# XiaoshuiHuang/GMF

Hardware: AMD Instinct MI355X
Metric: correspondences/sec (whole node) (higher is better)
Workload: dtype f32 (split-fp16 MFMA operands, fp32 accumulate; the cross products of the attention's two contractions, S = K Q'^T and O = P V, on block-scaled e4m3 operands wherever the device-side score guard allows)

## Files before the change

### gmf_amd/csrc/enc_common.hpp

```cpp
#pragma once
#include "mfma_core.hpp"
#include "launchers.hpp"
#include "kv_share_layout.hpp"

namespace gmf {

constexpr int C = 128;
constexpr int CF = C / 2;
constexpr int DH = 64;
constexpr int DHF = DH / 2;
constexpr int FFH = 512;
constexpr int kWavesPerWG = 4;

GMF_DEVINL void load_vec_block(float (&v)[16], const float* __restrict__ vec, int mb, int h) {
  const float4* p = reinterpret_cast<const float4*>(vec + 32 * mb) + h;
#pragma unroll
  for (int q = 0; q < 4; ++q) {
    const float4 t = p[2 * q];
    v[4 * q + 0] = t.x; v[4 * q + 1] = t.y; v[4 * q + 2] = t.z; v[4 * q + 3] = t.w;
  }
}

GMF_DEVINL void store_block_p32(float* __restrict__ tile_base, int mb, const float (&t)[16], int lane) {
  float4* p = reinterpret_cast<float4*>(tile_base) + (4 * mb) * 64 + lane;
// ... 209 lines not shown
  for (int s = 0; s < NS; ++s) mma3(acc, lw[(0 * NS + s) * 64], lw[(1 * NS + s) * 64], x.h[s], x.l[s]);
}

template <int NS>
GMF_DEVINL void mma_xw_h2(f32x16& acc, const f16x8* lw, const FragH2<NS>& x) {
#pragma unroll
  for (int s = 0; s < NS; ++s) mma3(acc, x.h[s], x.l[s], lw[(0 * NS + s) * 64], lw[(1 * NS + s) * 64]);
}

template <int NP>
GMF_DEVINL void mma_np(f32x16& acc, f16x8 ah, f16x8 al, f16x8 bh, f16x8 bl) {
  if (NP == 3) mma3(acc, ah, al, bh, bl);
  else acc = mfma_h16(ah, bh, acc);
}
template <int NS, int NP>
GMF_DEVINL void mma_wx_h2n(f32x16& acc, const f16x8* lw, const FragH2<NS>& x) {
#pragma unroll
  for (int s = 0; s < NS; ++s) {
    if (NP == 3) mma3(acc, lw[(0 * NS + s) * 64], lw[(1 * NS + s) * 64], x.h[s], x.l[s]);
    else acc = mfma_h16(lw[(0 * NS + s) * 64], x.h[s], acc);
  }
}
template <int NS, int NP>
GMF_DEVINL void mma_xw_h2n(f32x16& acc, const f16x8* lw, const FragH2<NS>& x) {
#pragma unroll
  for (int s = 0; s < NS; ++s) {
    if (NP == 3) mma3(acc, x.h[s], x.l[s], lw[(0 * NS + s) * 64], lw[(1 * NS + s) * 64]);
    else acc = mfma_h16(x.h[s], lw[(0 * NS + s) * 64], acc);
  }
}

GMF_DEVINL const f16x8* as_h2(const float4* p) { return reinterpret_cast<const f16x8*>(p); }

GMF_DEVINL float gelu_erf(float x) { return 0.5f * x * (1.0f + erff(x * 0.70710678118654752440f)); }

GMF_DEVINL float erf_bf(float a) {
  const float t = fabsf(a), s = a * a;
  float r = fmaf(-1.72853470e-5f, t, 3.83197126e-4f);
  const float u = fmaf(-3.88396438e-3f, t, 2.42546219e-2f);
  r = fmaf(r, s, u);
  r = fmaf(r, t, -1.06777877e-1f);
  r = fmaf(r, t, -6.34846687e-1f);
  r = fmaf(r, t, -1.28717512e-1f);
  r = fmaf(r, t, -t);
  const float big = 1.0f - __builtin_amdgcn_exp2f(r * 1.4426950408889634f);
  float q = -5.96761703e-4f;
  q = fmaf(q, s, 4.99119423e-3f);
  q = fmaf(q, s, -2.67681349e-2f);
  q = fmaf(q, s, 1.12819925e-1f);
  q = fmaf(q, s, -3.76125336e-1f);
  q = fmaf(q, s, 1.28379166e-1f);
  const float small = fmaf(q, t, t);
  return copysignf(t > 0.927734375f ? big : small, a);
}
GMF_DEVINL float gelu_erf_bf(float x) { return 0.5f * x * (1.0f + erf_bf(x * 0.70710678118654752440f)); }

GMF_DEVINL float gelu_erf_1r(float x) {
  const float ax = fabsf(x);
  const float t = fminf(ax * 0.70710678118654752440f, 4.3f);
  float p = 1.160468673e-05f;
  p = fmaf(p, t, -1.529631263e-04f);
  p = fmaf(p, t, 8.482293342e-04f);
  p = fmaf(p, t, -2.274774713e-03f);
  p = fmaf(p, t, 8.479235839e-05f);
  p = fmaf(p, t, 2.772448584e-02f);
  p = fmaf(p, t, -1.483079195e-01f);
  p = fmaf(p, t, -9.184429049e-01f);
  p = fmaf(p, t, -1.627907276e+00f);
  const float e = __builtin_amdgcn_exp2f(p * t);
  return fmaf(-0.5f * ax, e, fmaxf(x, 0.f));
}


GMF_DEVINL float len_diff(float a2, float b2) { return sqrt_cr(a2) - sqrt_cr(b2); }

GMF_DEVINL float compat_times(const float4* lp, int jl, const float (&si)[3], const float (&ti)[3], float inv_sig2, float sc) {
  const float4 a = lp[2 * jl], b = lp[2 * jl + 1];
  const float ax = si[0] - a.x, ay = si[1] - a.y, az = si[2] - a.z;
  const float bx = ti[0] - b.x, by = ti[1] - b.y, bz = ti[2] - b.z;
  const float d = len_diff(fmaf(az, az, fmaf(ay, ay, ax * ax)), fmaf(bz, bz, fmaf(by, by, bx * bx)));
  return fmaxf(1.0f - d * d * inv_sig2, 0.f) * sc;
}

constexpr int kJPerWave = 8;

constexpr int kCompatLdsFloats = 4 * 32 * 33;
template <int FMT>
GMF_DEVINL void compat_build_body(float* tr, const int I, const int by, const int pair, const float* __restrict__ pts8,
                                  float* __restrict__ c_dense, int N, int tiles, float inv_sig2, const PairTab* __restrict__ ptab) {
  const int lane = threadIdx.x & 63, h = lane >> 5, i = lane & 31;
  const int wave = __builtin_amdgcn_readfirstlane(threadIdx.x >> 6);
  const int tiles_p = (pair_rows(ptab, pair, N) + 31) >> 5;
  if (I >= tiles_p) return;
  const size_t pbase = (size_t)pair * tiles;
  float si[3], ti[3];
  {
    const float4* pp = reinterpret_cast<const float4*>(pts8 + (pbase * 32 + (size_t)I * 32 + i) * 8);
    const float4 a = pp[0], b = pp[1];
    si[0] = a.x; si[1] = a.y; si[2] = a.z; ti[0] = b.x; ti[1] = b.y; ti[2] = b.z;
  }
  constexpr int kTile16 = FMT ? 128 : 256;
  float4* const cbase = reinterpret_cast<float4*>(c_dense) + pbase * (size_t)tiles * kTile16 + lane;
  float4* const crow = cbase + (size_t)I * tiles * kTile16;
  auto store_tile = [&](float4* ct, const float (&c)[16]) {
    if (FMT == 1) {
#pragma unroll
      for (int q2 = 0; q2 < 2; ++q2) {
        f16x8 hv;
#pragma unroll
        for (int e = 0; e < 8; ++e) hv[e] = (_Float16)c[8 * q2 + e];
        ct[q2 * 64] = __builtin_bit_cast(float4, hv);
      }
    } else if (FMT == 2) {
#pragma unroll
      for (int q2 = 0; q2 < 2; ++q2) {
        unsigned wv[4];
        auto enc = [](float cv) { return (unsigned)__builtin_rintf(cv * 65535.0f); };
#pragma unroll
        for (int e = 0; e < 8; e += 2) wv[e >> 1] = enc(c[8 * q2 + e]) | (enc(c[8 * q2 + e + 1]) << 16);
        ct[q2 * 64] = make_float4(__uint_as_float(wv[0]), __uint_as_float(wv[1]), __uint_as_float(wv[2]), __uint_as_float(wv[3]));
      }
    } else {
#pragma unroll
      for (int q = 0; q < 4; ++q) ct[q * 64] = make_float4(c[4 * q], c[4 * q + 1], c[4 * q + 2], c[4 * q + 3]);
    }
  };
  float* const mt = tr + wave * 32 * 33;
  const int j0 = (by * 4 + wave) * kJPerWave;
  for (int J = max(j0, I); J < min(tiles_p, j0 + kJPerWave); ++J) {
    const float4* lp = reinterpret_cast<const float4*>(pts8 + (pbase * 32 + (size_t)J * 32) * 8) + 8 * h;
    float c[16];
#pragma unroll
    for (int r = 0; r < 16; ++r) c[r] = compat_times(lp, 8 * (r >> 2) + (r & 3), si, ti, inv_sig2, 1.0f);
    store_tile(crow + (size_t)J * kTile16, c);
    if (J > I) {
#pragma unroll
      for (int r = 0; r < 16; ++r) mt[i * 33 + 8 * (r >> 2) + 4 * h + (r & 3)] = c[r];
      asm volatile("s_waitcnt lgkmcnt(0)" ::: "memory");
      float d[16];
#pragma unroll
      for (int r = 0; r < 16; ++r) d[r] = mt[(8 * (r >> 2) + 4 * h + (r & 3)) * 33 + i];
      store_tile(cbase + ((size_t)J * tiles + I) * kTile16, d);
      asm volatile("s_waitcnt lgkmcnt(0)" ::: "memory");
    }
  }
}

GMF_DEVINL void pack_pts8_body(const long idx, const float* __restrict__ src, const float* __restrict__ tgt, float* __restrict__ dst,
                               int N, int Npad, long total, const PairTab* __restrict__ ptab, unsigned* __restrict__ zero_words,
                               int n_zero) {
  if (zero_words && idx < n_zero) zero_words[idx] = 0u;
  if (idx >= total) return;
  const int row = idx % Npad;
  const long b = idx / Npad;
  float4 a = make_float4(0.f, 0.f, 0.f, 0.f), c = a;
  if (row < pair_rows(ptab, (int)b, N)) {
    const size_t r0 = pair_row0(ptab, (int)b, N) + row;
    const float* ps = src + r0 * 3;
    const float* pt = tgt + r0 * 3;
    a = make_float4(ps[0], ps[1], ps[2], 0.f);
    c = make_float4(pt[0], pt[1], pt[2], 0.f);
  }
  reinterpret_cast<float4*>(dst)[2 * idx] = a;
  reinterpret_cast<float4*>(dst)[2 * idx + 1] = c;
}


}
```

### gmf_amd/csrc/encoder_kernels.hip

```cpp
#include <algorithm>
#include <type_traits>
#include "enc_common.hpp"
#include "enc_ff.hpp"

namespace gmf {

template <int MODE>
__global__ void __launch_bounds__(256, 2)
k_front(const float* __restrict__ in, const float* __restrict__ wst, const float* __restrict__ vecs,
        float* __restrict__ f_out, float* __restrict__ q_out, float* __restrict__ k_out,
        float* __restrict__ v_out, int N, int tiles) {
  __shared__ __attribute__((aligned(16))) float lds[2 * kStageFloats];
  const int lane = threadIdx.x & 63, wave = threadIdx.x >> 6, h = lane >> 5, i = lane & 31;
  const int pair = blockIdx.y;
  const int tile_raw = blockIdx.x * kWavesPerWG + wave;
  const bool active = tile_raw < tiles;
  const int tile = active ? tile_raw : tiles - 1;
  const size_t toff = ((size_t)pair * tiles + tile) * (32 * C);

  constexpr bool FIRST = (MODE == 1);
  StageStream ss;
  if (MODE == 2) ss.init(lds, lds + kStageFloats, wave, kWavesPerWG, lane, wst + 4 * kStageFloats, 12);
  else ss.init(lds, lds + kStageFloats, wave, kWavesPerWG, lane, wst, 16);
  ss.prime();
// ... 343 lines not shown
    for (int r = 0; r < 16; ++r) { x[r] = __builtin_amdgcn_exp2f(x[r] - m_off); ls += x[r]; }
    l_half = fmaf(l_half, alpha, ls);
    if (__any(moved)) {
#pragma unroll
      for (int db = 0; db < 4; ++db)
#pragma unroll
        for (int r = 0; r < 16; ++r) oacc[db][r] *= alpha;
    }
#pragma unroll
    for (int s2 = 0; s2 < 2; ++s2) {
      f16x8 ph, pl;
      split8h(&x[8 * s2], ph, pl);
#pragma unroll
      for (int db = 0; db < 4; ++db) {
        const int slot = 2 * db + s2;
        const f16x8 vh = lv[(0 * 8 + slot) * 64], vl = lv[(1 * 8 + slot) * 64];
        mma3(oacc[db], vh, vl, ph, pl);
      }
    }
  };
  for (int t = 0; t < tiles; t += 2) {
    tile_step(t, c_a, c_b);
    if (t + 1 < tiles) tile_step(t + 1, c_b, c_a);
  }

  float o[CF];
  {
    const float inv = 1.0f / xhalf_sum(l_half);
#pragma unroll
    for (int db = 0; db < 4; ++db)
#pragma unroll
      for (int r = 0; r < 16; ++r) o[16 * db + r] = oacc[db][r] * inv;
  }
  __syncthreads();
  StageStream ss;
  ss.init(lds, lds + kStageFloats, wave, WAVES, lane, wst, 5);
  ss.prime();
  float m1[DHF], m2[DHF];
#pragma unroll
  for (int mb = 0; mb < 2; ++mb) {
    const float4* lw = ss.acquire();
    f32x16 acc = zero16();
    mma_wx<CF>(acc, lw, o);
    float b[16];
    load_vec_block(b, vecs, mb, h);
#pragma unroll
    for (int r = 0; r < 16; ++r) m1[16 * mb + r] = relu_nan(acc[r] + b[r]);
  }
  {
    const float4* lw = ss.acquire();
#pragma unroll
    for (int mb = 0; mb < 2; ++mb) {
      f32x16 acc = zero16();
      mma_wx<DHF>(acc, lw + mb * (32 * DH / 4), m1);
      float b[16];
      load_vec_block(b, vecs + 64, mb, h);
#pragma unroll
      for (int r = 0; r < 16; ++r) m2[16 * mb + r] = relu_nan(acc[r] + b[r]);
    }
  }
#pragma unroll
  for (int st = 0; st < 2; ++st) {
    const float4* lw = ss.acquire();
#pragma unroll
    for (int hb = 0; hb < 2; ++hb) {
      const int mb = 2 * st + hb;
      f32x16 acc = zero16();
      mma_wx<DHF>(acc, lw + hb * (32 * DH / 4), m2);
      float b[16], fz[16], t[16];
      load_vec_block(b, vecs + 128, mb, h);
      load_block_p32(fz, fus + toff, mb, lane);
#pragma unroll
      for (int r = 0; r < 16; ++r) t[r] = acc[r] + b[r] + fz[r];
      if (active) store_block_p32(out + toff, mb, t, lane);
    }
  }
}

template <int FMT>
__global__ void __launch_bounds__(256)
k_compat_build(const float* __restrict__ pts8, float* __restrict__ c_dense, int N, int tiles, float inv_sig2,
               const PairTab* __restrict__ ptab) {
  __shared__ float tr[kCompatLdsFloats];
  compat_build_body<FMT>(tr, blockIdx.x, blockIdx.y, blockIdx.z, pts8, c_dense, N, tiles, inv_sig2, ptab);
}

GMF_DEVINL f32x16 mma3_part(int u, f32x16 acc, f16x8 ah, f16x8 al, f16x8 bh, f16x8 bl) {
  switch (u) {
    case 0: return mfma_h16(al, bh, acc);
    case 1: return mfma_h16(ah, bl, acc);
    default: return mfma_h16(ah, bh, acc);
  }
}


struct FusTile {
  const float* tile;
  GMF_DEVINL void load(float (&fz)[16], int mb, int lane, int h) const { load_block_p32(fz, tile, mb, lane); }
};

struct FusRegs {
  const float (&f)[CF];
  GMF_DEVINL void load(float (&fz)[16], int mb, int lane, int h) const {
#pragma unroll
    for (int r = 0; r < 16; ++r) fz[r] = f[16 * mb + r];
  }
};

constexpr int kTailVecFloats = 3 * C;
GMF_DEVINL void stage_tail_vecs(float* lvec, const float* __restrict__ vecs, const float* __restrict__ next_bias, int wave, int lane) {
  if (wave == 0) dma_piece_1k(vecs, lvec, lane);
  if (wave == 1 && next_bias && lane < 32) dma_piece_1k(next_bias, lvec + 2 * C, lane);
}

template <bool NEXT_PCN, class Stages, class Fus>
GMF_DEVINL void scattn_epilogue_h2(const float (&o)[CF], const bool active, Stages& ss, const float* __restrict__ vecs,
                                   const Fus& fus_tile, float* __restrict__ out_tile, const int lane, const int h,
                                   const float* __restrict__ next_bias = nullptr,
                                   unsigned* __restrict__ stat_next = nullptr, const int pair = 0, const bool row_valid = false) {
    FragH2<8> ox, featx;
    FragH2<4> m1x, m2x;
    if (active) ox.set(o);
#pragma unroll
    for (int mb = 0; mb < 2; ++mb) {
      const f16x8* lw = as_h2(ss.acquire());
      if (!active) continue;
      f32x16 acc = zero16();
      mma_wx_h2<8>(acc, lw, ox);
      float b[16], t1[16];
      load_vec_block(b, vecs, mb, h);
#pragma unroll
      for (int r = 0; r < 16; ++r) t1[r] = relu_nan(fmaf(acc[r], kH2Inv, b[r]));
      m1x.set_block(mb, t1);
    }
    {
      const f16x8* lw = as_h2(ss.acquire());
#pragma unroll
      for (int mb = 0; mb < 2; ++mb) {
        if (!active) continue;
        f32x16 acc = zero16();
        mma_wx_h2<4>(acc, lw + mb * (2 * 4 * 64), m1x);
        float b[16], t2[16];
        load_vec_block(b, vecs + 64, mb, h);
#pragma unroll
        for (int r = 0; r < 16; ++r) t2[r] = relu_nan(fmaf(acc[r], kH2Inv, b[r]));
        m2x.set_block(mb, t2);
      }
    }
#pragma unroll
    for (int st = 0; st < 2; ++st) {
      const f16x8* lw = as_h2(ss.acquire());
#pragma unroll
      for (int hb = 0; hb < 2; ++hb) {
        if (!active) continue;
        const int mb = 2 * st + hb;
        f32x16 acc = zero16();
        mma_wx_h2<4>(acc, lw + hb * (2 * 4 * 64), m2x);
        float b[16], fz[16], tt[16];
        load_vec_block(b, vecs + 128, mb, h);
        fus_tile.load(fz, mb, lane, h);
#pragma unroll
        for (int r = 0; r < 16; ++r) tt[r] = fmaf(acc[r], kH2Inv, b[r]) + fz[r];
        if (NEXT_PCN) featx.set_block(mb, tt);
        else if (active) store_block_p32(out_tile, mb, tt, lane);
      }
    }
    if (NEXT_PCN) {
// ... 1446 lines not shown
  const long b = bt / tiles;
  const int row = tile * 32 + (lane & 31);
  const int k0 = 8 * g + 4 * (lane >> 5);
  float4 v = make_float4(0.f, 0.f, 0.f, 0.f);
  if (row < pair_rows(ptab, (int)b, n_rows)) {
    const float* p = src + (ptab ? (long)ptab[b].row0 * sr : b * sb) + (long)row * sr + (long)k0 * sk;
    v = make_float4(p[0], p[sk], p[2 * sk], p[3 * sk]);
  }
  reinterpret_cast<float4*>(dst)[idx] = v;
}

__global__ void k_pack_rows_h2(const float* __restrict__ src, float* __restrict__ dst, int n_rows, int tiles, long total,
                               const PairTab* __restrict__ ptab, const float* __restrict__ copy_src, float* __restrict__ copy_dst,
                               long n_copy) {
  const long idx = (long)blockIdx.x * blockDim.x + threadIdx.x;
  if (idx < n_copy) copy_dst[idx] = copy_src[idx];
  if (idx >= total) return;
  const int lane = idx & 63, s8 = (idx >> 6) & 7;
  const long bt = idx >> 9;
  const int tile = bt % tiles;
  const int b = (int)(bt / tiles);
  const int h = lane >> 5, row = tile * 32 + (lane & 31);
  float v[8] = {0.f, 0.f, 0.f, 0.f, 0.f, 0.f, 0.f, 0.f};
  if (row < pair_rows(ptab, b, n_rows)) {
    const float* p = src + (pair_row0(ptab, b, n_rows) + row) * C + 32 * (s8 >> 1) + 16 * (s8 & 1) + 4 * h;
    const float4 a = *reinterpret_cast<const float4*>(p), c = *reinterpret_cast<const float4*>(p + 8);
    v[0] = a.x; v[1] = a.y; v[2] = a.z; v[3] = a.w; v[4] = c.x; v[5] = c.y; v[6] = c.z; v[7] = c.w;
  }
  f16x8 hi, lo;
  split8h(v, hi, lo);
  f16x8* out = reinterpret_cast<f16x8*>(dst + bt * kStageFloats);
  out[(0 * 8 + s8) * 64 + lane] = hi;
  out[(1 * 8 + s8) * 64 + lane] = lo;
}

__global__ void k_unpack_p32(const float* __restrict__ src, float* __restrict__ dst, int n_rows, int tiles, int K,
                             long sb, long sr, long sk, long total4, int* status) {
  const long idx = (long)blockIdx.x * blockDim.x + threadIdx.x;
  if (idx >= total4) return;
  const int lane = idx & 63;
  const long gi = idx >> 6;
  const int kg = K / 8;
  const int g = gi % kg;
  const long bt = gi / kg;
  const int tile = bt % tiles;
  const long b = bt / tiles;
  const int row = tile * 32 + (lane & 31);
  const int k0 = 8 * g + 4 * (lane >> 5);
  if (row < n_rows) {
    const float4 v = reinterpret_cast<const float4*>(src)[idx];
    float* p = dst + b * sb + (long)row * sr + (long)k0 * sk;
    p[0] = v.x; p[sk] = v.y; p[2 * sk] = v.z; p[3 * sk] = v.w;
    if (status && (not_finite(v.x) || not_finite(v.y) || not_finite(v.z) || not_finite(v.w)))
      __hip_atomic_fetch_or(status, 1, __ATOMIC_RELAXED, __HIP_MEMORY_SCOPE_SYSTEM);
  }
}

__global__ void k_pack_pts8(const float* __restrict__ src, const float* __restrict__ tgt, float* __restrict__ dst,
                            int N, int Npad, long total, const PairTab* __restrict__ ptab, unsigned* __restrict__ zero_words,
                            int n_zero) {
  pack_pts8_body((long)blockIdx.x * blockDim.x + threadIdx.x, src, tgt, dst, N, Npad, total, ptab, zero_words, n_zero);
}

}


#include "launchers.hpp"

namespace gmf {

static inline dim3 tile_grid(int tiles, int B, int sets = 1) { return dim3((tiles + kWavesPerWG - 1) / kWavesPerWG, B, sets); }

hipError_t launch_front(int mode, const float* in, const float* wst, const float* vecs, float* f, float* q, float* k,
                        float* v, int B, int N, int tiles, hipStream_t s) {
  const dim3 g = tile_grid(tiles, B);
  if (mode == 1) hipLaunchKernelGGL(k_front<1>, g, dim3(256), 0, s, in, wst, vecs, f, q, k, v, N, tiles);
  else if (mode == 2) hipLaunchKernelGGL(k_front<2>, g, dim3(256), 0, s, in, wst, vecs, f, q, k, v, N, tiles);
  else hipLaunchKernelGGL(k_front<0>, g, dim3(256), 0, s, in, wst, vecs, f, q, k, v, N, tiles);
  return hipGetLastError();
}

hipError_t launch_compat_build(const float* pts8, float* c_dense, int B, int N, int tiles, float sigma_d, int fmt, hipStream_t s,
                               const PairTab* ptab) {
  const dim3 grid(tiles, (tiles + 4 * kJPerWave - 1) / (4 * kJPerWave), B);
  const float inv = 1.0f / (sigma_d * sigma_d);
  if (fmt == 1) hipLaunchKernelGGL(k_compat_build<1>, grid, dim3(256), 0, s, pts8, c_dense, N, tiles, inv, ptab);
  else if (fmt == 2) hipLaunchKernelGGL(k_compat_build<2>, grid, dim3(256), 0, s, pts8, c_dense, N, tiles, inv, ptab);
  else hipLaunchKernelGGL(k_compat_build<0>, grid, dim3(256), 0, s, pts8, c_dense, N, tiles, inv, ptab);
  return hipGetLastError();
}

hipError_t launch_scattn_fp32(const float* q, const float* k, const float* v, const float* pts8, const float* fus,
                              const float* wst, const float* vecs, float* out, int B, int N, int tiles, float sigma_d,
                              hipStream_t s) {
  hipLaunchKernelGGL(k_scattn<false>, tile_grid(tiles, B), dim3(256), 0, s, q, k, v, pts8, fus, wst, vecs, out, N, tiles,
                     1.0f / (sigma_d * sigma_d));
  return hipGetLastError();
}

hipError_t launch_small_attn_ff_merge(bool tile_merge, const float* q, const float* k, const float* v, const float* x1, float* ff_part,
                                      int ff_hs, float* out, int B, int N, int tiles, int ksplits, const ForwardBuffers& fb,
                                      const LayerRun& lr, hipStream_t s) {
  const int wpp = (tiles + 3) / 4, W = wpp * B;
  const int per_xcd = (W >> 3) + ((W & 7) ? 1 : 0);
  const int n_attn = 8 * per_xcd * ksplits, n_ff = W * ff_hs;
  const float *ff_wst = lr.w.ff_wst_h2, *ff_vecs = lr.w.ff_vec;
  auto go = [&](auto kern, bool pvf8) {
    hipLaunchKernelGGL(kern, dim3(n_attn + n_ff), dim3(256), 0, s, n_attn, q, k, v, lr.epi_wst, lr.epi_vec, N, tiles, wpp, fb.dense, W,
                       ksplits, fb.part_o, fb.part_ml, x1, ff_wst, ff_vecs, ff_part, B, ff_hs, pvf8 ? (const unsigned*)fb.v_scale : nullptr,
                       pvf8 ? lr.guard : PvGuard{}, fb.ptab);
  };
  if (fb.fmt == 2 && fb.v_scale) go(k_small_attn_ff<2, true>, true);
  else if (fb.fmt == 2) go(k_small_attn_ff<2>, false);
  else if (fb.v_scale) go(k_small_attn_ff<0, true>, true);
  else go(k_small_attn_ff<0>, false);
  if (tile_merge)
    hipLaunchKernelGGL(k_scattn_merge_tile, dim3(tiles, B), dim3(256), 0, s, fb.part_o, fb.part_ml, lr.epi_wst, lr.epi_vec, out,
                       tiles, ksplits, lr.epi_next_wst, lr.epi_next_bias, (const float*)ff_part, ff_hs, x1, ff_vecs + 2 * C + 2 * FFH,
                       lr.guard.stat_next, N, fb.ptab);
  else
    hipLaunchKernelGGL(k_scattn_merge, dim3(8 * per_xcd), dim3(256), 0, s, fb.part_o, fb.part_ml, x1, lr.epi_wst, lr.epi_vec, out,
                       tiles, wpp, W, 0, ksplits, lr.epi_next_wst, lr.epi_next_bias, (const float*)ff_part, ff_hs, x1,
                       ff_vecs + 2 * C + 2 * FFH, lr.guard.stat_next, N, fb.ptab);
  return hipGetLastError();
}

hipError_t launch_scattn_h2p(const float* q, const float* k, const float* v, const float* fus, float* out, int B, int N, int tiles,
                             const ForwardBuffers& fb, const LayerRun& lr, int n_full, int ksplits, hipStream_t s) {
  const float* const vecs = lr.epi_vec;
  const int wpp = (tiles + 3) / 4, W = wpp * B;
  const int per_xcd = (W >> 3) + ((W & 7) ? 1 : 0);
  const int max_tail = std::max(0, per_xcd - n_full);
  const dim3 grid(8 * (std::min(n_full, per_xcd) + max_tail * ksplits));
  auto go = [&](auto kern, bool pvf8) {
    hipLaunchKernelGGL(kern, grid, dim3(256), 0, s, q, k, v, fus, lr.epi_wst, vecs, out, N, tiles, wpp, fb.dense, W, n_full, ksplits,
                       fb.part_o, fb.part_ml, lr.epi_next_wst, lr.epi_next_bias, fb.ptab, pvf8 ? (const unsigned*)fb.v_scale : nullptr, lr.qf_img,
                       lr.qw_wst, lr.qw_bias, pvf8 ? lr.guard : PvGuard{}, lr.kvf_vec, fb.dense_fb);
  };
  const bool pvf8 = fb.v_scale != nullptr, fold = lr.kvf_vec != nullptr;
  if (fb.half && max_tail == 0)
    hipLaunchKernelGGL(k_scattn_fast, dim3(8 * per_xcd), dim3(256), 0, s, q, k, v, fus, lr.epi_wst, vecs, out, N, tiles, wpp, fb.dense, W,
                       lr.epi_next_wst, lr.epi_next_bias);
  else if (fb.half)
    go(k_scattn_h2p<1, 1>, false);
  else if (fb.fmt == 2 && fb.dense_fb && pvf8)
    fold ? go(k_scattn_h2p<3, 2, true, true, 0>, true) : go(k_scattn_h2p<3, 2, true, false, 0>, true);
  else if (fb.fmt == 2 && pvf8)
    fold ? go(k_scattn_h2p<3, 2, true, true>, true) : go(k_scattn_h2p<3, 2, true>, true);
  else if (fb.fmt == 2)
    fold ? go(k_scattn_h2p<3, 2, false, true>, false) : go(k_scattn_h2p<3, 2>, false);
  else if (pvf8)
    fold ? go(k_scattn_h2p<3, 0, true, true>, true) : go(k_scattn_h2p<3, 0, true>, true);
  else
    fold ? go(k_scattn_h2p<3, 0, false, true>, false) : go(k_scattn_h2p<3, 0>, false);
  if (max_tail > 0)
    hipLaunchKernelGGL(k_scattn_merge, dim3(8 * max_tail), dim3(256), 0, s, fb.part_o, fb.part_ml, fus, lr.epi_wst, vecs, out,
                       tiles, wpp, W, n_full, ksplits, lr.epi_next_wst, lr.epi_next_bias, (const float*)nullptr, 0,
                       (const float*)nullptr, (const float*)nullptr, lr.guard.stat_next, N, fb.ptab);
  return hipGetLastError();
}

hipError_t launch_scattn_h2(const float* q, const float* k, const float* v, const float* pts8, const float* fus, const float* wst,
                            const float* vecs, float* out, int B, int N, int tiles, float sigma_d, hipStream_t s, const float* c_dense) {
  const float inv = 1.0f / (sigma_d * sigma_d);
  const int wpp = (tiles + 3) / 4;
  if (c_dense) hipLaunchKernelGGL(k_scattn_h2<true>, dim3(wpp * B), dim3(256), 0, s, q, k, v, pts8, fus, wst, vecs, out, N, tiles, inv, wpp, c_dense);
  else hipLaunchKernelGGL(k_scattn_h2<false>, dim3(wpp * B), dim3(256), 0, s, q, k, v, pts8, fus, wst, vecs, out, N, tiles, inv, wpp, c_dense);
// ... 81 lines not shown
```

### gmf_amd/csrc/mfma_core.hpp

```cpp
#pragma once
#include <hip/hip_runtime.h>
#include <stdint.h>

#include "launchers.hpp"

#define GMF_DEVINL __device__ __forceinline__

namespace gmf {

GMF_DEVINL int pair_rows(const PairTab* pt, int pair, int N) { return pt ? pt[pair].n : N; }
GMF_DEVINL size_t pair_row0(const PairTab* pt, int pair, int N) { return pt ? (size_t)pt[pair].row0 : (size_t)pair * N; }

typedef float f32x16 __attribute__((ext_vector_type(16)));
typedef float f32x4 __attribute__((ext_vector_type(4)));

constexpr int kWave = 64;
constexpr int kTileRows = 32;
constexpr int kStageFloats = 4096;

GMF_DEVINL f32x16 mfma32(float a, float b, f32x16 c) {
  return __builtin_amdgcn_mfma_f32_32x32x2f32(a, b, c, 0, 0, 0);
}

typedef float f32x2 __attribute__((ext_vector_type(2)));
// ... 97 lines not shown
}
GMF_DEVINL float relu_nan(float x) { return x < 0.f ? 0.f : x; }
GMF_DEVINL bool not_finite(float v) { return !(__builtin_fabsf(v) <= 3.4028234e38f); }

GMF_DEVINL f32x16 zero16() {
  f32x16 z;
#pragma unroll
  for (int r = 0; r < 16; ++r) z[r] = 0.f;
  return z;
}

template <int KF>
GMF_DEVINL void mma_wx(f32x16& acc, const float4* lw, const float (&x)[KF]) {
#pragma unroll
  for (int g = 0; g < KF / 4; ++g) {
    const float4 w = lw[g * 64];
    acc = mfma32(w.x, x[4 * g + 0], acc);
    acc = mfma32(w.y, x[4 * g + 1], acc);
    acc = mfma32(w.z, x[4 * g + 2], acc);
    acc = mfma32(w.w, x[4 * g + 3], acc);
  }
}

template <int KF>
GMF_DEVINL void mma_xw(f32x16& acc, const float4* lw, const float (&x)[KF]) {
#pragma unroll
  for (int g = 0; g < KF / 4; ++g) {
    const float4 w = lw[g * 64];
    acc = mfma32(x[4 * g + 0], w.x, acc);
    acc = mfma32(x[4 * g + 1], w.y, acc);
    acc = mfma32(x[4 * g + 2], w.z, acc);
    acc = mfma32(x[4 * g + 3], w.w, acc);
  }
}

GMF_DEVINL int frag_feature(int r, int h) { return 8 * (r >> 2) + 4 * h + (r & 3); }

template <int KF>
GMF_DEVINL void load_vec_frag(float (&v)[KF], const float* __restrict__ vec, int h) {
  const float4* p = reinterpret_cast<const float4*>(vec) + h;
#pragma unroll
  for (int g = 0; g < KF / 4; ++g) {
    const float4 t = p[2 * g];
    v[4 * g + 0] = t.x; v[4 * g + 1] = t.y; v[4 * g + 2] = t.z; v[4 * g + 3] = t.w;
  }
}

template <int KF>
GMF_DEVINL void load_frag_p32(float (&x)[KF], const float* __restrict__ tile_base, int lane) {
  const float4* p = reinterpret_cast<const float4*>(tile_base) + lane;
#pragma unroll
  for (int g = 0; g < KF / 4; ++g) {
    const float4 t = p[g * 64];
    x[4 * g + 0] = t.x; x[4 * g + 1] = t.y; x[4 * g + 2] = t.z; x[4 * g + 3] = t.w;
  }
}

template <int KF>
GMF_DEVINL void store_frag_p32(float* __restrict__ tile_base, const float (&x)[KF], int lane) {
  float4* p = reinterpret_cast<float4*>(tile_base) + lane;
#pragma unroll
  for (int g = 0; g < KF / 4; ++g) p[g * 64] = make_float4(x[4 * g + 0], x[4 * g + 1], x[4 * g + 2], x[4 * g + 3]);
}

template <int KF>
GMF_DEVINL void load_row_frag_p32(float (&x)[KF], const float* __restrict__ pair_base, int row, int n_rows, int h) {
  if (row >= 0 && row < n_rows) {
    const float4* p = reinterpret_cast<const float4*>(pair_base) + (size_t)(row >> 5) * (KF / 4) * 64 + h * 32 + (row & 31);
#pragma unroll
    for (int g = 0; g < KF / 4; ++g) {
      const float4 t = p[g * 64];
      x[4 * g + 0] = t.x; x[4 * g + 1] = t.y; x[4 * g + 2] = t.z; x[4 * g + 3] = t.w;
    }
  } else {
#pragma unroll
    for (int k = 0; k < KF; ++k) x[k] = 0.f;
  }
}

GMF_DEVINL float sqrt_cr(float x) {
  const float y = __builtin_amdgcn_sqrtf(x);
  const float hr = 0.5f * __builtin_amdgcn_rsqf(fmaxf(x, 1e-36f));
  return fmaf(fmaf(-y, y, x), hr, y);
}


GMF_DEVINL float xhalf_sum(float v) { return v + __shfl_xor(v, 32, 64); }
GMF_DEVINL float xhalf_max(float v) { return fmaxf(v, __shfl_xor(v, 32, 64)); }
GMF_DEVINL float xhalf_max_swap(float v) {
  const auto r = __builtin_amdgcn_permlane32_swap(__float_as_uint(v), __float_as_uint(v), false, false);
  return __builtin_fmaxf(__uint_as_float(r[0]), __uint_as_float(r[1]));
}

template <int KF>
GMF_DEVINL void layernorm_frag(float (&y)[KF], const float (&x)[KF], const float* __restrict__ gamma,
                               const float* __restrict__ beta, int h) {
  float s = 0.f;
#pragma unroll
  for (int k = 0; k < KF; ++k) s += x[k];
  const float mu = xhalf_sum(s) * (1.0f / (2 * KF));
  float v = 0.f;
#pragma unroll
  for (int k = 0; k < KF; ++k) { const float d = x[k] - mu; v = fmaf(d, d, v); }
  const float rstd = rsqrtf(xhalf_sum(v) * (1.0f / (2 * KF)) + 1e-5f);
  const float4* pg = reinterpret_cast<const float4*>(gamma) + h;
  const float4* pb = reinterpret_cast<const float4*>(beta) + h;
#pragma unroll
  for (int g = 0; g < KF / 4; ++g) {
    const float4 ga = pg[2 * g], be = pb[2 * g];
    y[4 * g + 0] = fmaf((x[4 * g + 0] - mu) * rstd, ga.x, be.x);
    y[4 * g + 1] = fmaf((x[4 * g + 1] - mu) * rstd, ga.y, be.y);
    y[4 * g + 2] = fmaf((x[4 * g + 2] - mu) * rstd, ga.z, be.z);
    y[4 * g + 3] = fmaf((x[4 * g + 3] - mu) * rstd, ga.w, be.w);
  }
}

GMF_DEVINL void dma_piece_1k(const float* __restrict__ gsrc_piece, float* lds_piece, int lane) {
  __builtin_amdgcn_global_load_lds(
      (const void __attribute__((address_space(1)))*)(gsrc_piece + lane * 4),
      (void __attribute__((address_space(3)))*)(lds_piece), 16, 0, 0);
}

GMF_DEVINL void dma_piece_1k_s(const float* __restrict__ gsrc_piece_uniform, float* lds_piece, unsigned lane_off16) {
  unsigned keep;
  const unsigned lds_dst = (unsigned)(uintptr_t)(void __attribute__((address_space(3)))*)(lds_piece);
  asm volatile("s_mov_b32 %0, m0\n\ts_mov_b32 m0, %3\n\ts_nop 0\n\tglobal_load_lds_dwordx4 %1, %2\n\ts_mov_b32 m0, %0"
               : "=&s"(keep) : "v"(lane_off16), "s"(gsrc_piece_uniform), "s"(lds_dst) : "memory");
}

GMF_DEVINL void dma_4k_s(const float* __restrict__ gsrc_uniform, float* lds_dst_base, unsigned lane_off16) {
  unsigned keep;
  const unsigned lds_dst = (unsigned)(uintptr_t)(void __attribute__((address_space(3)))*)(lds_dst_base);
  asm volatile("s_mov_b32 %0, m0\n\ts_mov_b32 m0, %3\n\ts_nop 0\n\t"
               "global_load_lds_dwordx4 %1, %2\n\tglobal_load_lds_dwordx4 %1, %2 offset:1024\n\t"
               "global_load_lds_dwordx4 %1, %2 offset:2048\n\tglobal_load_lds_dwordx4 %1, %2 offset:3072\n\ts_mov_b32 m0, %0"
               : "=&s"(keep) : "v"(lane_off16), "s"(gsrc_uniform), "s"(lds_dst) : "memory");
}

GMF_DEVINL void dma_2k_s(const float* __restrict__ gsrc_uniform, float* lds_dst_base, unsigned lane_off16) {
  unsigned keep;
  const unsigned lds_dst = (unsigned)(uintptr_t)(void __attribute__((address_space(3)))*)(lds_dst_base);
  asm volatile("s_mov_b32 %0, m0\n\ts_mov_b32 m0, %3\n\ts_nop 0\n\t"
               "global_load_lds_dwordx4 %1, %2\n\tglobal_load_lds_dwordx4 %1, %2 offset:1024\n\ts_mov_b32 m0, %0"
               : "=&s"(keep) : "v"(lane_off16), "s"(gsrc_uniform), "s"(lds_dst) : "memory");
}

typedef __fp16 h16x4_tr __attribute__((__vector_size__(8)));
GMF_DEVINL f16x8 lds_read_tr16x8(unsigned addr_a, unsigned addr_b) {
  typedef _Float16 f16x4v __attribute__((ext_vector_type(4)));
  const f16x4v a = __builtin_bit_cast(f16x4v, __builtin_amdgcn_ds_read_tr16_b64_v4f16(
      (h16x4_tr __attribute__((address_space(3)))*)(uintptr_t)addr_a));
  const f16x4v b = __builtin_bit_cast(f16x4v, __builtin_amdgcn_ds_read_tr16_b64_v4f16(
      (h16x4_tr __attribute__((address_space(3)))*)(uintptr_t)addr_b));
  return __builtin_shufflevector(a, b, 0, 1, 2, 3, 4, 5, 6, 7);
}
GMF_DEVINL f16x8 lds_read_f16x8(unsigned addr) {
  return *(const f16x8 __attribute__((address_space(3)))*)(uintptr_t)addr;
}

GMF_DEVINL void dma_vec(const float* __restrict__ gsrc, float* lds_dst, int n_floats, int wave, int n_waves, int lane) {
  for (int p = wave; p * 256 < n_floats; p += n_waves)
    if (p * 256 + lane * 4 < n_floats) dma_piece_1k(gsrc + p * 256, lds_dst + p * 256, lane);
}

GMF_DEVINL void dma_issue(const float* __restrict__ gsrc, float* lds_dst, int n_pieces, int wave, int n_waves, int lane) {
  for (int p = wave; p < n_pieces; p += n_waves) dma_piece_1k(gsrc + p * 256, lds_dst + p * 256, lane);
// ... 96 lines not shown
```

Measured before the change: 10.90 million.

## Pair row tiles per block in compat build and cheapen sqrt and u16 encode

The compatibility-matrix builder now has each block handle two adjacent row tiles: each half-wave takes one row tile, and the two results are exchanged with permlane32_swap so each wave writes two full output tiles. This halves the grid in x and halves kJPerWave. The sqrt drops the hardware sqrt and uses a single rsq plus one Newton step. The u16 quantisation uses a magic-number add instead of rintf, and the LDS transpose for the mirrored tile now works on packed 16-bit words. The aim is to cut ALU work per element and per-tile overhead, at the risk of small numerical differences and trickier index logic.

```diff
diff --git a/gmf_amd/csrc/enc_common.hpp b/gmf_amd/csrc/enc_common.hpp
--- a/gmf_amd/csrc/enc_common.hpp
+++ b/gmf_amd/csrc/enc_common.hpp
@@ -315,7 +315,25 @@
   return fmaxf(1.0f - d * d * inv_sig2, 0.f) * sc;
 }
 
-constexpr int kJPerWave = 8;
+constexpr int kJPerWave = 4;
+
+GMF_DEVINL float len_diff1(float a2, float b2) { return sqrt_cr1(a2) - sqrt_cr1(b2); }
+GMF_DEVINL float compat_elem(const float4 a, const float4 b, const float (&si)[3], const float (&ti)[3], float inv_sig2) {
+  const float ax = si[0] - a.x, ay = si[1] - a.y, az = si[2] - a.z;
+  const float bx = ti[0] - b.x, by = ti[1] - b.y, bz = ti[2] - b.z;
+  const float d = len_diff1(fmaf(az, az, fmaf(ay, ay, ax * ax)), fmaf(bz, bz, fmaf(by, by, bx * bx)));
+  return fmaxf(1.0f - d * d * inv_sig2, 0.f);
+}
+
+GMF_DEVINL unsigned enc_u16_bits(float c) {
+#pragma clang fp contract(off)
+  return __float_as_uint(c * 65535.0f + 8388608.0f);
+}
+template <int FMT>
+GMF_DEVINL unsigned pack_c16(float c0, float c1) {
+  if (FMT == 1) { const f16x2 hv = {(_Float16)c0, (_Float16)c1}; return __builtin_bit_cast(unsigned, hv); }
+  return __builtin_amdgcn_perm(enc_u16_bits(c1), enc_u16_bits(c0), 0x05040100u);
+}
 
 constexpr int kCompatLdsFloats = 4 * 32 * 33;
 template <int FMT>
@@ -324,57 +342,73 @@
   const int lane = threadIdx.x & 63, h = lane >> 5, i = lane & 31;
   const int wave = __builtin_amdgcn_readfirstlane(threadIdx.x >> 6);
   const int tiles_p = (pair_rows(ptab, pair, N) + 31) >> 5;
-  if (I >= tiles_p) return;
+  if ((I & 1) || I >= tiles_p) return;
+  const bool two = I + 1 < tiles_p;
   const size_t pbase = (size_t)pair * tiles;
   float si[3], ti[3];
   {
-    const float4* pp = reinterpret_cast<const float4*>(pts8 + (pbase * 32 + (size_t)I * 32 + i) * 8);
+    const float4* pp = reinterpret_cast<const float4*>(pts8 + (pbase * 32 + (size_t)(two ? I + h : I) * 32 + i) * 8);
     const float4 a = pp[0], b = pp[1];
     si[0] = a.x; si[1] = a.y; si[2] = a.z; ti[0] = b.x; ti[1] = b.y; ti[2] = b.z;
   }
   constexpr int kTile16 = FMT ? 128 : 256;
+  constexpr int kWords = FMT ? 8 : 16;
   float4* const cbase = reinterpret_cast<float4*>(c_dense) + pbase * (size_t)tiles * kTile16 + lane;
   float4* const crow = cbase + (size_t)I * tiles * kTile16;
-  auto store_tile = [&](float4* ct, const float (&c)[16]) {
-    if (FMT == 1) {
-#pragma unroll
-      for (int q2 = 0; q2 < 2; ++q2) {
-        f16x8 hv;
-#pragma unroll
-        for (int e = 0; e < 8; ++e) hv[e] = (_Float16)c[8 * q2 + e];
-        ct[q2 * 64] = __builtin_bit_cast(float4, hv);
+  auto store_tile = [&](float4* ct, const unsigned (&w)[kWords]) {
+#pragma unroll
+    for (int q = 0; q < kWords / 4; ++q)
+      ct[q * 64] = make_float4(__uint_as_float(w[4 * q]), __uint_as_float(w[4 * q + 1]), __uint_as_float(w[4 * q + 2]), __uint_as_float(w[4 * q + 3]));
+  };
+  unsigned* const mt = reinterpret_cast<unsigned*>(tr) + wave * 32 * 33;
+  auto mirror_tile = [&](float4* ct, const unsigned (&w)[kWords]) {
+    unsigned d[kWords];
+    if (FMT == 0) {
+#pragma unroll
+      for (int r = 0; r < 16; ++r) mt[i * 33 + 8 * (r >> 2) + 4 * h + (r & 3)] = w[r];
+      asm volatile("s_waitcnt lgkmcnt(0)" ::: "memory");
+#pragma unroll
+      for (int r = 0; r < 16; ++r) d[r] = mt[(8 * (r >> 2) + 4 * h + (r & 3)) * 33 + i];
+    } else {
+#pragma unroll
+      for (int m = 0; m < 8; ++m) mt[i * 17 + 4 * (m >> 1) + 2 * h + (m & 1)] = w[m];
+      asm volatile("s_waitcnt lgkmcnt(0)" ::: "memory");
+      const unsigned short* m16 = reinterpret_cast<const unsigned short*>(mt);
+#pragma unroll
+      for (int m = 0; m < 8; ++m) {
+        const int jl = 8 * (m >> 1) + 4 * h + 2 * (m & 1);
+        d[m] = (unsigned)m16[jl * 34 + i] | ((unsigned)m16[(jl + 1) * 34 + i] << 16);
       }
-    } else if (FMT == 2) {
-#pragma unroll
-      for (int q2 = 0; q2 < 2; ++q2) {
-        unsigned wv[4];
-        auto enc = [](float cv) { return (unsigned)__builtin_rintf(cv * 65535.0f); };
-#pragma unroll
-        for (int e = 0; e < 8; e += 2) wv[e >> 1] = enc(c[8 * q2 + e]) | (enc(c[8 * q2 + e + 1]) << 16);
-        ct[q2 * 64] = make_float4(__uint_as_float(wv[0]), __uint_as_float(wv[1]), __uint_as_float(wv[2]), __uint_as_float(wv[3]));
-      }
-    } else {
-#pragma unroll
-      for (int q = 0; q < 4; ++q) ct[q * 64] = make_float4(c[4 * q], c[4 * q + 1], c[4 * q + 2], c[4 * q + 3]);
-    }
+    }
+    store_tile(ct, d);
+    asm volatile("s_waitcnt lgkmcnt(0)" ::: "memory");
   };
-  float* const mt = tr + wave * 32 * 33;
   const int j0 = (by * 4 + wave) * kJPerWave;
   for (int J = max(j0, I); J < min(tiles_p, j0 + kJPerWave); ++J) {
-    const float4* lp = reinterpret_cast<const float4*>(pts8 + (pbase * 32 + (size_t)J * 32) * 8) + 8 * h;
-    float c[16];
-#pragma unroll
-    for (int r = 0; r < 16; ++r) c[r] = compat_times(lp, 8 * (r >> 2) + (r & 3), si, ti, inv_sig2, 1.0f);
-    store_tile(crow + (size_t)J * kTile16, c);
-    if (J > I) {
-#pragma unroll
-      for (int r = 0; r < 16; ++r) mt[i * 33 + 8 * (r >> 2) + 4 * h + (r & 3)] = c[r];
-      asm volatile("s_waitcnt lgkmcnt(0)" ::: "memory");
-      float d[16];
-#pragma unroll
-      for (int r = 0; r < 16; ++r) d[r] = mt[(8 * (r >> 2) + 4 * h + (r & 3)) * 33 + i];
-      store_tile(cbase + ((size_t)J * tiles + I) * kTile16, d);
-      asm volatile("s_waitcnt lgkmcnt(0)" ::: "memory");
+    const float4* kq = reinterpret_cast<const float4*>(pts8 + (pbase * 32 + (size_t)J * 32) * 8);
+    unsigned x[kWords], y[kWords];
+#pragma unroll
+    for (int g = 0; g < 4; ++g) {
+      float cx[4], cy[4];
+#pragma unroll
+      for (int e = 0; e < 4; ++e) {
+        cx[e] = compat_elem(kq[2 * (8 * g + e)], kq[2 * (8 * g + e) + 1], si, ti, inv_sig2);
+        cy[e] = compat_elem(kq[2 * (8 * g + 4 + e)], kq[2 * (8 * g + 4 + e) + 1], si, ti, inv_sig2);
+      }
+#pragma unroll
+      for (int e = 0; e < (FMT ? 2 : 4); ++e) {
+        const unsigned xa = FMT ? pack_c16<FMT>(cx[2 * e], cx[2 * e + 1]) : __float_as_uint(cx[e]);
+        const unsigned ya = FMT ? pack_c16<FMT>(cy[2 * e], cy[2 * e + 1]) : __float_as_uint(cy[e]);
+        const auto sw = __builtin_amdgcn_permlane32_swap(xa, ya, false, false);
+        x[(FMT ? 2 : 4) * g + e] = sw[0];
+        y[(FMT ? 2 : 4) * g + e] = sw[1];
+      }
+    }
+    store_tile(crow + (size_t)J * kTile16, x);
+    if (two) store_tile(crow + ((size_t)tiles + J) * kTile16, y);
+    if (J > I + 1) {
+      mirror_tile(cbase + ((size_t)J * tiles + I) * kTile16, x);
+      if (two) mirror_tile(cbase + ((size_t)J * tiles + I + 1) * kTile16, y);
     }
   }
 }
diff --git a/gmf_amd/csrc/encoder_kernels.hip b/gmf_amd/csrc/encoder_kernels.hip
--- a/gmf_amd/csrc/encoder_kernels.hip
+++ b/gmf_amd/csrc/encoder_kernels.hip
@@ -449,7 +449,7 @@
 k_compat_build(const float* __restrict__ pts8, float* __restrict__ c_dense, int N, int tiles, float inv_sig2,
                const PairTab* __restrict__ ptab) {
   __shared__ float tr[kCompatLdsFloats];
-  compat_build_body<FMT>(tr, blockIdx.x, blockIdx.y, blockIdx.z, pts8, c_dense, N, tiles, inv_sig2, ptab);
+  compat_build_body<FMT>(tr, 2 * blockIdx.x, blockIdx.y, blockIdx.z, pts8, c_dense, N, tiles, inv_sig2, ptab);
 }
 
 GMF_DEVINL f32x16 mma3_part(int u, f32x16 acc, f16x8 ah, f16x8 al, f16x8 bh, f16x8 bl) {
@@ -2062,7 +2062,7 @@
 
 hipError_t launch_compat_build(const float* pts8, float* c_dense, int B, int N, int tiles, float sigma_d, int fmt, hipStream_t s,
                                const PairTab* ptab) {
-  const dim3 grid(tiles, (tiles + 4 * kJPerWave - 1) / (4 * kJPerWave), B);
+  const dim3 grid((tiles + 1) / 2, (tiles + 4 * kJPerWave - 1) / (4 * kJPerWave), B);
   const float inv = 1.0f / (sigma_d * sigma_d);
   if (fmt == 1) hipLaunchKernelGGL(k_compat_build<1>, grid, dim3(256), 0, s, pts8, c_dense, N, tiles, inv, ptab);
   else if (fmt == 2) hipLaunchKernelGGL(k_compat_build<2>, grid, dim3(256), 0, s, pts8, c_dense, N, tiles, inv, ptab);
diff --git a/gmf_amd/csrc/mfma_core.hpp b/gmf_amd/csrc/mfma_core.hpp
--- a/gmf_amd/csrc/mfma_core.hpp
+++ b/gmf_amd/csrc/mfma_core.hpp
@@ -203,6 +203,11 @@
   const float y = __builtin_amdgcn_sqrtf(x);
   const float hr = 0.5f * __builtin_amdgcn_rsqf(fmaxf(x, 1e-36f));
   return fmaf(fmaf(-y, y, x), hr, y);
+}
+GMF_DEVINL float sqrt_cr1(float x) {
+  const float r = __builtin_amdgcn_rsqf(fmaxf(x, 0x1p-126f));
+  const float y = x * r;
+  return fmaf(fmaf(-y, y, x), 0.5f * r, y);
 }
 
 
```

Result: no change. 10.98 million (median of 6 runs) (+0.8%).
